# SDU-Gary/PCSS-Unet

Hardware: AMD Instinct MI355X
Metric: frames/sec 7x512x512 U-Net fwd+bwd (train step) (higher is better)
Workload: dtype f32; 1 GPU; configs[1]: batch=8/GPU 7x512x512 fp32 train step (fwd + 0.9*L1 + bwd + RCCL grad all-reduce + clip + AdamW); global_batch=8, in_ch=7, parallelism=dp1

## Files before the change

include/nsm.h:

```cpp
#ifndef NSM_H_
#define NSM_H_

#include <stddef.h>
#include <stdint.h>

#ifdef __cplusplus
extern "C" {
#endif

#define NSM_OK 0
#define NSM_E_ARG 1
#define NSM_E_HIP 2
#define NSM_E_WS 3

#define NSM_F32 0
#define NSM_BF16 1
#define NSM_F16 2

#define NSM_AMAX_WORDS 2048
#define NSM_PACK_FWD 0
#define NSM_PACK_DGRAD 1

int nsm_version(void);
int nsm_get_last_error(char* buf, size_t n);
// ... 62 lines not shown
int nsm_wino_output_bf16(const float* Mb, int B, int H, int W, int cout_p, int tile,
                         const float* bias, void* y, int ldy, float* partial, int nslot,
                         void* stream);
int nsm_wino_dual_f16(const void* dy, int lddy, int B, int H, int W, int c_p, int tile, void* V,
                      void* dM, const uint32_t* amax_dy, void* stream);
int nsm_wino_dual_bn_f16(const void* g, int ldg, const void* y, int ldy, int B, int H, int W, int c_p,
                         int tile, const float* scale, const float* shift, float slope,
                         const float* mask, const float* mean, const float* coef, void* V, void* dM,
                         const uint32_t* bound, void* stream);
int nsm_wino_gemm_f16m(const void* V, const void* U, int B, int H, int W, int cin_p, int cout_p,
                       int tile, void* M16, int* m16e, const uint32_t* amax_v, float beta_v,
                       const uint32_t* amax_u, float beta_u, void* stream);
int nsm_wino_output_bf16m(const void* M16, const int* m16e, int B, int H, int W, int cin_p,
                          int cout_p, int tile, const uint32_t* amax_v, float beta_v,
                          const uint32_t* amax_u, float beta_u, const float* bias, void* y, int ldy,
                          float* partial, int nslot, void* stream);
int nsm_wino_output_bf16m_act(const void* M16, const int* m16e, int B, int H, int W, int cin_p,
                              int cout_p, int tile, const uint32_t* amax_v, float beta_v,
                              const uint32_t* amax_u, float beta_u, const float* bias, void* y,
                              int ldy, const float* act_scale, const float* act_shift, float slope,
                              void* stream);
int nsm_wino_dout_f16(const void* dy, int lddy, int B, int H, int W, int c_p, int tile, void* dM,
                      const uint32_t* amax_dy, void* stream);
size_t nsm_wino_wgrad_f16_ws(int B, int H, int W, int cin_p, int cout_p, int tile);
int nsm_conv3x3_wgrad_wino_f16(const void* dM, const void* V, int B, int H, int W, int cin_p,
                               int cout_p, int cin, int cout, int tile, float* dw, float* ws,
                               size_t ws_floats, const uint32_t* amax_dy, const uint32_t* amax_x,
                               void* stream);
int nsm_wino_dual_input_bn_h2(const float* g, int ldg, const float* y, int ldy, int B, int H, int W,
                              int c_p, int tile, const float* scale, const float* shift,
                              float slope, const float* mask, const float* mean, const float* coef,
                              void* Vh, void* dMh, const uint32_t* bound, void* stream);
size_t nsm_wino_wgrad_h2_ws(int B, int H, int W, int cin_p, int cout_p, int tile);
int nsm_conv3x3_wgrad_wino_h2(const void* dMh, const void* Vh, int B, int H, int W, int cin_p,
                              int cout_p, int cin, int cout, int tile, float* dw, float* ws,
                              size_t ws_floats, const uint32_t* amax_dy, const uint32_t* amax_x,
                              void* stream);
int nsm_wino_gemm_h2(const void* V, const void* U, int B, int H, int W, int cin_p, int cout_p,
                     int tile, float* Mb, const uint32_t* amax_v, float beta_v,
                     const uint32_t* amax_u, float beta_u, void* stream);
int nsm_wino_gemm_h2_plan(int B, int H, int W, int cin_p, int cout_p, int tile, int* plan);
int nsm_wino_wgrad_h2_plan(int B, int H, int W, int cin_p, int cout_p, int tile, int* plan);
int nsm_conv1x1_h2_rows(int M, int N, int K, int bnbwd);
int nsm_conv1x1_h2(const void* xh, int M, int cin_p, const void* wh, const float* bias, int cout_p,
                   float* y, int ldy, float* stats, const uint32_t* amax_x,
                   const uint32_t* amax_w, void* stream);
int nsm_conv1x1_dgrad_bnbwd_h2(const void* dy2h, int M, int cop, const void* w2dh, int cip,
                               const float* y1, int ldy1, const float* scale, const float* shift,
                               const float* mean, const float* invstd, const float* mask, int HW,
                               float slope, int mode, float* partial, const float* coef,
                               float* out, int ldo, const uint32_t* amax_dy2,
                               const uint32_t* amax_w, uint32_t* amax_out, uint32_t* amax_k1dz,
                               void* stream);
size_t nsm_conv1x1_wgrad_h2_ws(int M, int cin_p, int cout_p);
int nsm_conv1x1_wgrad_h2(const void* dyh, const void* xh, int M, int cin_p, int cout_p, int cin,
                         int cout, float* dw, float* ws, size_t ws_floats, const uint32_t* amax_dy,
                         const uint32_t* amax_x, void* stream);
int nsm_conv3x3_h2_rows(int M, int N);
int nsm_conv3x3_h2(const void* xh, int B, int H, int W, int cin_p, const void* wh,
                   const float* bias, int cout_p, float* y, int ldy, float* stats,
                   const uint32_t* amax_x, const uint32_t* amax_w, void* stream);
size_t nsm_conv3x3_wgrad_h2_ws(int B, int H, int W, int cin_p, int cout_p);
int nsm_conv3x3_wgrad_h2(const void* dyh, const void* xh, int B, int H, int W, int cin_p,
                         int cout_p, int cin, int cout, float* dw, float* ws, size_t ws_floats,
                         const uint32_t* amax_dy, const uint32_t* amax_x, void* stream);
int nsm_set_f32_split(int mode);
int nsm_wino_output(const float* Mb, int B, int H, int W, int cout_p, int tile, const float* bias,
                    float* y, int ldy, void* stream);
int nsm_wino_output_stats(const float* Mb, int B, int H, int W, int cout_p, int tile,
                          const float* bias, float* y, int ldy, float* partial, int nslot,
                          void* stream);
int nsm_wino_stat_slots(int B, int H, int W, int cout_p, int tile);
int nsm_wino_stat_step(int cout_p, int tile);

size_t nsm_wino_wgrad_ws(int B, int H, int W, int cin_p, int cout_p, int tile);
int nsm_conv3x3_wgrad_wino(const float* dy, int lddy, const float* V, int B, int H, int W,
                           int cin_p, int cout_p, int cin, int cout, int tile, float* dw,
                           float* ws, size_t ws_floats, void* stream);
int nsm_wino_dual_input(const float* dy, int lddy, int B, int H, int W, int c_p, int tile,
                        float* V, float* dM, uint32_t* amax_v, uint32_t* amax_dm, void* stream);
int nsm_wino_dual_input_bn(const float* g, int ldg, const float* y, int ldy, int B, int H, int W,
                           int c_p, int tile, const float* scale, const float* shift, float slope,
                           const float* mask, const float* mean, const float* coef, float* V,
                           float* dM, uint32_t* amax_v, uint32_t* amax_dm, void* stream);
int nsm_conv3x3_wgrad_wino_dm(const float* dM, const float* V, int B, int H, int W, int cin_p,
                              int cout_p, int cin, int cout, int tile, float* dw, float* ws,
                              size_t ws_floats, const uint32_t* amax_dm, const uint32_t* amax_v,
                              void* stream);

size_t nsm_conv_wgrad_ws(int B, int H, int W, int cin_p, int cout_p, int ksize);
int nsm_conv_wgrad(const float* dy, int lddy, const float* x, int ldx, int B, int H, int W,
                   int cin_p, int cout_p, int ksize, const float* pro_scale, const float* pro_shift,
                   const float* pro_mask, float slope, float* ws, size_t ws_floats, int cin, int cout,
                   float* dw, const uint32_t* amax_dy, const uint32_t* amax_x, void* stream);

int nsm_reduce_chunks(int M, int C);
int nsm_reduce_rows(int M, int C);
int nsm_bn_stats(const void* y, int ld, int M, int C, float* partial, int nchunk, int dtype,
                 void* stream);
int nsm_bn_finalize_train(const float* partial, int nchunk, int rows_per_chunk, int M, int C,
                          int c_real,
                          const float* gamma, const float* beta, float* run_mean, float* run_var,
                          int64_t* num_batches, float momentum, float eps, int n_updates,
                          float* mean, float* invstd, float* scale, float* shift, uint32_t* bound,
                          float bound_mul, void* stream);
int nsm_bn_partials_merge(const float* partial, int nchunk, int rows_per_chunk, int M, int C,
// ... 296 lines not shown
```

pcss-unet_amd/csrc/nsm_conv_h2d.inc:

```

struct EpiStoreH {
  using P = EpiStoreP;
  template <int TM, int TN, int WM, int WN>
  static constexpr int lds_bytes() {
    constexpr int a = WM * WN * 32 * (TN * 32 + 4) * 4, b = WM * WN * TN * 32 * 4;
    return a > b ? a : b;
  }
  template <int TM, int TN, int WM, int WN>
  __device__ static void apply(const P& e, f32x16 (&acc)[TM][TN], const EpiCtx& cx, int M, int N,
                               int) {
    const int col = cx.lane & 31, h = cx.lane >> 5;
#pragma unroll
    for (int tn = 0; tn < TN; ++tn) {
      const int n = cx.nb + tn * 32 + col;
      const float bv = (e.bias && n < N) ? e.bias[n] : 0.f;
#pragma unroll
      for (int tm = 0; tm < TM; ++tm)
#pragma unroll
        for (int i = 0; i < 16; ++i) acc[tm][tn][i] += bv;
    }
    constexpr int WC = TN * 32, WCP = WC + 4, CPR = WC / 4;
    float* reg = cx.lds + (cx.wm * WN + cx.wn) * (32 * WCP);
#pragma unroll
    for (int tm = 0; tm < TM; ++tm) {
// ... 46 lines not shown
static bool h2d_nfast() { static const bool v = env_flag("NSM_H2D_NFAST", true); return v; }

template <int BM, int BN, int WM, int WN, class EP>
static int launch_h2d(const H2RowsP& ap, const H2RowsP& bp, const typename EP::P& ep, int M, int N,
                      int K, H2Scale sa, H2Scale sb, hipStream_t s) {
  constexpr int NW = WM * WN;
  const dim3 grid(ceil_div(M, BM), ceil_div(N, BN), 1);
  const long long total = (long long)grid.x * grid.y;
  const int remap = h2d_nfast() && grid.y > 1 && total % 8 == 0 ? 2 : 0;
  hipLaunchKernelGGL((gemm_h2_kernel<BM, BN, WM, WN, H2RowsDma<BM, NW>, H2RowsDma<BN, NW>, EP>), grid,
                     dim3(NW * 64), 0, s, ap, bp, ep, M, N, K, K, 1, remap, sa, sb);
  NSM_LAUNCH_CHECK("conv1x1_h2");
  return 0;
}

template <class EP>
static int gemm_h2d(int tile, const H2RowsP& ap, const H2RowsP& bp, const typename EP::P& ep, int M,
                    int N, int K, H2Scale sa, H2Scale sb, hipStream_t s) {
  switch (tile) {
    case 1:
      if constexpr (!std::is_same<EP, EpiBnBwd>::value)
        return launch_h2d<256, 256, 2, 4, EP>(ap, bp, ep, M, N, K, sa, sb, s);
      return fail(NSM_E_ARG, "conv1x1_h2: tile");
    case 2: return launch_h2d<256, 128, 4, 2, EP>(ap, bp, ep, M, N, K, sa, sb, s);
    case 3: return launch_h2d<128, 128, 2, 2, EP>(ap, bp, ep, M, N, K, sa, sb, s);
    case 4: return launch_h2d<256, 64, 4, 1, EP>(ap, bp, ep, M, N, K, sa, sb, s);
    case 5: return launch_h2d<128, 64, 2, 2, EP>(ap, bp, ep, M, N, K, sa, sb, s);
    default: return launch_h2d<128, 32, 4, 1, EP>(ap, bp, ep, M, N, K, sa, sb, s);
  }
}

static WgradPlan plan_wgrad_h2(long long px, int cin_p, int cout_p) {
  WgradPlan pl;
  pl.BM = cout_p >= 128 ? 128 : (cout_p >= 64 ? 64 : 32);
  pl.BN = cin_p >= 128 ? 128 : (cin_p >= 64 ? 64 : 32);
  const long long tiles = (long long)ceil_div(cout_p, pl.BM) * ceil_div(cin_p, pl.BN);
  static const long long target = env_int("NSM_H2D_WG_BLOCKS", 512);
  long long sp = target / tiles;
  const long long maxs = (px + 255) / 256;
  long long slab_cap = (128ll << 20) / ((long long)cout_p * cin_p);
  if (slab_cap < 1) slab_cap = 1;
  if (sp > maxs) sp = maxs;
  if (sp > slab_cap) sp = slab_cap;
  if (sp > 512) sp = 512;
  if (sp < 1) sp = 1;
  long long kc = (px + sp - 1) / sp;
  kc = (kc + 31) / 32 * 32;
  sp = (px + kc - 1) / kc;
  pl.splits = (int)sp;
  pl.kchunk = (int)kc;
  pl.ws_floats = (size_t)sp * cout_p * cin_p;
  if (sp > 16) pl.ws_floats += (size_t)((sp + 15) / 16) * cout_p * cin_p;
  return pl;
}

extern "C" int nsm_conv1x1_h2_rows(int M, int N, int K, int bnbwd) {
  return h2d_tile_bm(h2d_tile(M, N, K, bnbwd != 0));
}

extern "C" int nsm_conv1x1_h2(const void* xh, int M, int cin_p, const void* wh, const float* bias,
                              int cout_p, float* y, int ldy, float* stats, const uint32_t* amax_x,
                              const uint32_t* amax_w, void* stream) {
  NSM_CHECK_ARG(xh && wh && y && amax_x && amax_w, "conv1x1_h2: null pointer");
  NSM_CHECK_ARG(M > 0 && cin_p % 32 == 0 && cout_p % 32 == 0 && ldy >= cout_p && ldy % 4 == 0,
                "conv1x1_h2: bad shape");
  NSM_CHECK_ARG(((uintptr_t)xh % 16) == 0 && ((uintptr_t)wh % 16) == 0 && ((uintptr_t)y % 16) == 0,
                "conv1x1_h2: 16-B alignment");
  NSM_CHECK_ARG((long long)M * 2 * cin_p < (1ll << 30), "conv1x1_h2: operand too large");
  const int K = 2 * cin_p;
  H2RowsP ap{(const bf16_t*)xh, K, M, 0};
  H2RowsP bp{(const bf16_t*)wh, K, cout_p, 0};
  EpiStoreP ep{y, ldy, bias, stats, 0, nullptr, nullptr, 0.f, nullptr, 0, 1};
  return gemm_h2d<EpiStoreH>(h2d_tile(M, cout_p, K, false), ap, bp, ep, M, cout_p, K,
                             H2Scale{amax_x, 1.f}, H2Scale{amax_w, 1.f}, as_stream(stream));
}

extern "C" int nsm_conv1x1_dgrad_bnbwd_h2(const void* dy2h, int M, int cop, const void* w2dh,
                                          int cip, const float* y1, int ldy1, const float* scale,
                                          const float* shift, const float* mean,
                                          const float* invstd, const float* mask, int HW,
                                          float slope, int mode, float* partial, const float* coef,
                                          float* out, int ldo, const uint32_t* amax_dy2,
                                          const uint32_t* amax_w, uint32_t* amax_out,
                                          uint32_t* amax_k1dz, void* stream) {
  NSM_CHECK_ARG(dy2h && w2dh && y1 && scale && shift && mean && amax_dy2 && amax_w,
                "conv1x1_dgrad_bnbwd_h2: null pointer");
  NSM_CHECK_ARG(mode >= 0 && mode <= 2, "conv1x1_dgrad_bnbwd_h2: mode %d", mode);
  NSM_CHECK_ARG(mode == 2 || (partial && invstd), "conv1x1_dgrad_bnbwd_h2: modes 0/1 need partials");
  NSM_CHECK_ARG(mode == 0 || out, "conv1x1_dgrad_bnbwd_h2: modes 1/2 need an output");
  NSM_CHECK_ARG(mode != 2 || coef, "conv1x1_dgrad_bnbwd_h2: mode 2 needs coef");
  NSM_CHECK_ARG(M > 0 && HW > 0 && cop % 32 == 0 && cip % 32 == 0 && ldy1 >= cip && ldy1 % 4 == 0 &&
                    (mode == 0 || (ldo >= cip && ldo % 4 == 0)),
                "conv1x1_dgrad_bnbwd_h2: bad shape");
  NSM_CHECK_ARG(((uintptr_t)dy2h % 16) == 0 && ((uintptr_t)w2dh % 16) == 0 &&
                    ((uintptr_t)y1 % 16) == 0 && ((uintptr_t)out % 16) == 0,
                "conv1x1_dgrad_bnbwd_h2: 16-B alignment");
  NSM_CHECK_ARG((long long)M * 2 * cop < (1ll << 30), "conv1x1_dgrad_bnbwd_h2: operand too large");
  BnBwdEpiP ep{out, ldo, y1, ldy1, scale, shift, mean, invstd, coef, mask,
               make_fastdiv((uint32_t)HW), slope, partial, mode};
  if (mode == 2) ep.amax = amax_out;
  else ep.k1dz = amax_k1dz;
  const int K = 2 * cop;
  H2RowsP ap{(const bf16_t*)dy2h, K, M, 0};
  H2RowsP bp{(const bf16_t*)w2dh, K, cip, 0};
  return gemm_h2d<EpiBnBwd>(h2d_tile(M, cip, K, true), ap, bp, ep, M, cip, K, H2Scale{amax_dy2, 1.f},
                            H2Scale{amax_w, 1.f}, as_stream(stream));
}

extern "C" size_t nsm_conv1x1_wgrad_h2_ws(int M, int cin_p, int cout_p) {
  return plan_wgrad_h2(M, cin_p, cout_p).ws_floats;
}

extern "C" int nsm_conv1x1_wgrad_h2(const void* dyh, const void* xh, int M, int cin_p, int cout_p,
                                    int cin, int cout, float* dw, float* ws, size_t ws_floats,
                                    const uint32_t* amax_dy, const uint32_t* amax_x, void* stream) {
  NSM_CHECK_ARG(dyh && xh && dw && ws && amax_dy && amax_x, "conv1x1_wgrad_h2: null pointer");
  NSM_CHECK_ARG(M > 0 && cin_p % 32 == 0 && cout_p % 32 == 0 && cin <= cin_p && cout <= cout_p,
                "conv1x1_wgrad_h2: bad shape");
  NSM_CHECK_ARG(((uintptr_t)dyh % 16) == 0 && ((uintptr_t)xh % 16) == 0 && ((uintptr_t)ws % 16) == 0,
                "conv1x1_wgrad_h2: 16-B alignment");
  NSM_CHECK_ARG((long long)M * 2 * std::max(cin_p, cout_p) < (1ll << 30),
                "conv1x1_wgrad_h2: operand too large");
  const WgradPlan pl = plan_wgrad_h2(M, cin_p, cout_p);
  if (ws_floats < pl.ws_floats)
    return fail(NSM_E_WS, "conv1x1_wgrad_h2: workspace %zu < %zu floats", ws_floats, pl.ws_floats);
  hipStream_t s = as_stream(stream);
  const int rc = wino_wgrad_gemm_h2((const bf16_t*)dyh, (const bf16_t*)xh, M, cin_p, cout_p, 1,
                                    pl.BM, pl.BN, pl.kchunk, pl.splits, ws, H2Scale{amax_dy, 1.f},
                                    H2Scale{amax_x, 1.f}, s);
  if (rc) return rc;
  return wgrad_finish(ws, pl, cout_p, cin_p, cin_p, 1, cin, cout, dw, s);
}

template <int R, int NW>
struct H2ConvDma : ConvActDma<R, NW, 64> {
  static constexpr int KT = 64;
  __device__ void init(const ConvActPB& p, int m0, int kb, int ke, int wid, int lane, int) {
    ConvActDma<R, NW, 64>::init(p, m0, kb, ke, wid, lane);
  }
};
template <int R, int NW>
struct H2RowsKDma : RowsKDma<R, NW, 64> {
  static constexpr int KT = 64;
  __device__ void init(const RowsKPB& p, int n0, int kb, int ke, int wid, int lane, int) {
    RowsKDma<R, NW, 64>::init(p, n0, kb, ke, wid, lane);
  }
};
template <int R, int NW>
struct H2ShiftDma : PixRowsDma<R, NW, true, 32> {
  static constexpr int KT = 32;
  int kb0;
  __device__ void init(const PixRowsPB& p, int off, int kb, int ke, int wid, int lane, int) {
    kb0 = kb;
    PixRowsDma<R, NW, true, 32>::init(p, 2 * off, kb, ke, wid, lane);
  }
  __device__ void prep(const PixRowsPB& p, int krel) { PixRowsDma<R, NW, true, 32>::prep(p, kb0 + krel); }
};

static ConvActPB h2_conv_operand(const void* xh, int B, int H, int W, int cin_p) {
// ... 114 lines not shown
```

pcss-unet_amd/nsm_amd/_lib.py:

```python
import ctypes
import os

import torch

_HERE = os.path.dirname(os.path.abspath(__file__))
LIB_PATH = os.environ.get("NSM_LIB", os.path.join(_HERE, "libnsm.so"))

P = ctypes.c_void_p
I = ctypes.c_int
L = ctypes.c_int64
F = ctypes.c_float
Z = ctypes.c_size_t
D = ctypes.c_double
U64 = ctypes.c_uint64

_SIGS = {
    "nsm_version": (I, []),
    "nsm_get_last_error": (I, [ctypes.c_char_p, Z]),
    "nsm_pack_conv_weight": (I, [P, I, I, I, I, I, I, P, P]),
    "nsm_pad_vec": (I, [P, I, I, P, P]),
    "nsm_conv_fwd": (I, [P, I, I, I, I, I, P, P, I, I, P, I, P, P, P, F, P]),
    "nsm_conv_stat_rows": (I, [I, I, I, I]),
    "nsm_conv_fwd_stats": (I, [P, I, I, I, I, I, P, P, I, I, P, I, P, P, P, F, P, P, P, P]),
    "nsm_wino_ws": (Z, [I, I, I, I, I, I]),
    "nsm_wino_weight": (I, [P, I, I, I, I, I, I, P, P]),
    "nsm_conv3x3_wino": (I, [P, I, I, I, I, I, P, P, I, I, I, P, I, P, Z, P]),
    "nsm_wino_input": (I, [P, I, I, I, I, I, I, I, P, P]),
    "nsm_wino_gemm": (I, [P, P, I, I, I, I, I, I, P, P]),
    "nsm_wino_gemm_s": (I, [P, P, I, I, I, I, I, I, P, P, P, P]),
    "nsm_absmax": (I, [P, L, P, P]),
    "nsm_zero_u32": (I, [P, L, P]),
    "nsm_absmax_bf16": (I, [P, L, P, P]),
    "nsm_pmc_calib": (I, [I, P, P, L, P]),
    "nsm_to_h2": (I, [P, L, I, P, F, P, P]),
    "nsm_wino_gemm_h2": (I, [P, P, I, I, I, I, I, I, P, P, F, P, F, P]),
    "nsm_wino_gemm_h2_plan": (I, [I, I, I, I, I, I, P]),
    "nsm_wino_wgrad_h2_plan": (I, [I, I, I, I, I, I, P]),
    "nsm_wino_beta": (F, [I, I]),
    "nsm_wino_input_h2": (I, [P, I, I, I, I, I, I, I, I, P, P, P]),
    "nsm_wino_dual_input_h2": (I, [P, I, I, I, I, I, I, P, P, P, P]),
    "nsm_wino_dual_input_bn_h2": (I, [P, I, P, I, I, I, I, I, I, P, P, F, P, P, P, P, P, P, P]),
    "nsm_wino_input_f16": (I, [P, I, I, I, I, I, I, P, P, P]),
    "nsm_wino_input_f16_resize": (I, [P, I, I, I, I, I, I, I, I, P, P, P]),
    "nsm_wino_gemm_f16": (I, [P, P, I, I, I, I, I, I, P, P, F, P, F, P]),
    "nsm_wino_output_bf16": (I, [P, I, I, I, I, I, P, P, I, P, I, P]),
    "nsm_wino_gemm_f16m": (I, [P, P, I, I, I, I, I, I, P, P, P, F, P, F, P]),
    "nsm_wino_output_bf16m": (I, [P, P, I, I, I, I, I, I, P, F, P, F, P, P, I, P, I, P]),
    "nsm_wino_output_bf16m_act": (I, [P, P, I, I, I, I, I, I, P, F, P, F, P, P, I, P, P, F, P]),
    "nsm_wino_dout_f16": (I, [P, I, I, I, I, I, I, P, P, P]),
    "nsm_wino_dual_f16": (I, [P, I, I, I, I, I, I, P, P, P, P]),
    "nsm_wino_dual_bn_f16": (I, [P, I, P, I, I, I, I, I, I, P, P, F, P, P, P, P, P, P, P]),
    "nsm_wino_wgrad_f16_ws": (Z, [I, I, I, I, I, I]),
    "nsm_conv3x3_wgrad_wino_f16": (I, [P, P, I, I, I, I, I, I, I, I, P, P, Z, P, P, P]),
    "nsm_wino_wgrad_h2_ws": (Z, [I, I, I, I, I, I]),
    "nsm_conv3x3_wgrad_wino_h2": (I, [P, P, I, I, I, I, I, I, I, I, P, P, Z, P, P, P]),
    "nsm_set_f32_split": (I, [I]),
    "nsm_wino_output": (I, [P, I, I, I, I, I, P, P, I, P]),
    "nsm_wino_wgrad_ws": (Z, [I, I, I, I, I, I]),
    "nsm_conv3x3_wgrad_wino": (I, [P, I, P, I, I, I, I, I, I, I, I, P, P, Z, P]),
    "nsm_conv_wgrad_ws": (Z, [I, I, I, I, I, I]),
    "nsm_conv_wgrad": (I, [P, I, P, I, I, I, I, I, I, I, P, P, P, F, P, Z, I, I, P, P, P, P]),
    "nsm_reduce_chunks": (I, [I, I]),
    "nsm_reduce_rows": (I, [I, I]),
    "nsm_bn_stats": (I, [P, I, I, I, P, I, I, P]),
    "nsm_bn_finalize_train": (I, [P, I, I, I, I, I, P, P, P, P, P, F, F, I, P, P, P, P, P, F, P]),
    "nsm_bn_act_h2": (I, [P, I, I, I, P, P, F, P, I, P, P, P]),
    "nsm_conv1x1_h2_rows": (I, [I, I, I, I]),
    "nsm_conv1x1_h2": (I, [P, I, I, P, P, I, P, I, P, P, P, P]),
    "nsm_conv1x1_dgrad_bnbwd_h2": (I, [P, I, I, P, I, P, I, P, P, P, P, P, I, F, I, P, P, P, I, P,
                                       P, P, P, P]),
    "nsm_conv3x3_h2_rows": (I, [I, I]),
    "nsm_conv3x3_h2": (I, [P, I, I, I, I, P, P, I, P, I, P, P, P, P]),
    "nsm_conv3x3_wgrad_h2_ws": (Z, [I, I, I, I, I]),
    "nsm_conv3x3_wgrad_h2": (I, [P, P, I, I, I, I, I, I, I, P, P, Z, P, P, P]),
    "nsm_input_prep_h2": (I, [P, I, I, I, I, P, I, P, P]),
    "nsm_conv1x1_wgrad_h2_ws": (Z, [I, I, I]),
    "nsm_conv1x1_wgrad_h2": (I, [P, P, I, I, I, I, I, P, P, Z, P, P, P]),
    "nsm_bn_partials_merge": (I, [P, I, I, I, I, I, P, P]),
    "nsm_bn_finalize_eval": (I, [P, P, P, P, I, I, F, P, P, P, P, P]),
    "nsm_bn_act": (I, [P, I, I, I, P, P, F, P, I, P, I, P, I, I, P, P]),
    "nsm_bn_bwd_reduce": (I, [P, I, P, I, I, I, I, P, P, F, P, P, P, P, I, I, P, P]),
    "nsm_bn_bwd_finalize": (I, [P, I, I, I, I, P, P, P, P, P, P, P, P, P]),
    "nsm_bn_bwd_apply_h2": (I, [P, I, P, I, I, I, I, P, P, F, P, P, P, P, P, P]),
    "nsm_bn_bwd_apply": (I, [P, I, P, I, I, I, I, P, P, F, P, P, P, P, I, I, P, P]),
    "nsm_sum_rows": (I, [P, I, I, I, P, P]),
    "nsm_resize_fwd_act": (I, [P, I, I, I, I, P, I, I, P, P, F, P, I, P]),
    "nsm_up2_resize_fwd_act": (I, [P, I, I, I, I, P, I, I, P, P, F, P, I, P]),
    "nsm_bn_act_pool": (I, [P, I, I, I, I, P, P, F, P, P, I, P, P]),
    "nsm_wino_dual_input": (I, [P, I, I, I, I, I, I, P, P, P, P, P]),
    "nsm_wino_dual_input_bn": (I, [P, I, P, I, I, I, I, I, I, P, P, F, P, P, P, P, P, P, P, P]),
    "nsm_conv3x3_wgrad_wino_dm": (I, [P, P, I, I, I, I, I, I, I, I, P, P, Z, P, P, P]),
    "nsm_conv_fwd_act": (I, [P, I, I, I, I, I, P, P, I, I, P, I, P, P, F, P, I, I, P]),
    "nsm_wino_output_act": (I, [P, I, I, I, I, I, P, P, I, P, P, F, P, I, P]),
    "nsm_bnred_chunks": (I, [I, I, I, I, I]),
    "nsm_avgpool2_bwd_add_bnred": (I, [P, I, I, I, I, P, P, I, P, P, P, P, P, F, P, P, P]),
    "nsm_resize_bwd_bnred": (I, [P, I, I, I, I, P, I, I, I, P, P, P, P, P, F, P, P, P]),
    "nsm_up2_resize_bwd_bnred": (I, [P, I, I, I, I, P, I, I, I, P, P, P, P, P, F, P, P, P]),
    "nsm_wino_input_resize": (I, [P, I, I, I, I, I, I, I, I, I, P, P, P]),
    "nsm_wino_output_stats": (I, [P, I, I, I, I, I, P, P, I, P, I, P]),
    "nsm_wino_stat_slots": (I, [I, I, I, I, I]),
    "nsm_wino_stat_step": (I, [I, I]),
    "nsm_conv1x1_bnbwd_chunks": (I, [I, I, I, I, I, I]),
    "nsm_conv1x1_dgrad_bnbwd": (I, [P, I, I, I, I, I, P, I, P, I, P, P, P, P, P, F, I, P, P, P, I,
                                    I, P, P, P, P]),
    "nsm_avgpool2_fwd": (I, [P, I, I, I, I, P, I, P]),
    "nsm_avgpool2_bwd_add": (I, [P, I, I, I, I, P, P, I, P]),
    "nsm_resize_fwd": (I, [P, I, I, I, I, P, I, I, I, P]),
    "nsm_resize_bwd": (I, [P, I, I, I, I, P, I, I, I, P]),
    "nsm_up2_resize_fwd": (I, [P, I, I, I, I, P, I, I, I, P]),
    "nsm_up2_resize_bwd": (I, [P, I, I, I, I, P, I, I, I, P]),
    "nsm_input_prep": (I, [P, I, I, I, I, P, I, I, P, P]),
    "nsm_input_grad": (I, [P, I, I, I, I, I, P, I, P]),
    "nsm_head_fwd": (I, [P, I, I, I, I, P, P, P, I, P]),
    "nsm_head_bwd_blocks": (I, [I, I, I]),
    "nsm_head_bwd": (I, [P, P, P, I, I, I, I, P, P, P, P, P, I, P]),
    "nsm_loss_blocks": (I, [L]),
    "nsm_l1_loss_fwd": (I, [P, P, L, F, P, P, P]),
    "nsm_expdiff_mean": (I, [P, P, L, F, P, P, P]),
    "nsm_l1_loss_bwd": (I, [P, P, L, F, P, P, I, P]),
    "nsm_detail_blocks": (I, [I, I, I]),
    "nsm_detail_loss_fwd": (I, [P, P, I, I, I, F, F, F, P, P, P, P]),
    "nsm_detail_loss_bwd": (I, [P, P, I, I, I, F, F, F, P, P, P, I, P]),
    "nsm_ssim_blocks": (I, [I, I, I]),
# ... 133 lines not shown
```

pcss-unet_amd/nsm_amd/ops.py:

```python
import os

import torch

from ._lib import call, ptr, stream

F32 = torch.float32
BF16 = torch.bfloat16
F16S = torch.int16
PACK_FWD, PACK_DGRAD = 0, 1
NSM_F32, NSM_BF16, NSM_F16 = 0, 1, 2
S16 = (BF16, F16S)


def dt(t):
    if t.dtype == BF16:
        return NSM_BF16
    if t.dtype == F16S:
        return NSM_F16
    if t.dtype != F32:
        raise TypeError(f"activations must be float32, bfloat16 or f16 storage (int16), "
                        f"got {t.dtype}")
    return NSM_F32


# ... 312 lines not shown
             ptr(amax[0]), bv, ptr(amax[1]), bu, st)
    else:
        call("nsm_wino_gemm_f16", ptr(V), ptr(U), B, H, W, cin_p, cout_p, 4, ptr(Mb), ptr(amax[0]),
             bv, ptr(amax[1]), bu, st)
    if evg is not None:
        evg.record()
    if not keep_v:
        V = None
    y = torch.empty(B * H * W, cout_p, dtype=BF16, device=x.device)
    if act is not None:
        assert not stats
        call("nsm_wino_output_bf16m_act", ptr(Mb), ptr(m16e), B, H, W, cin_p, cout_p, 4,
             ptr(amax[0]), bv, ptr(amax[1]), bu, ptr(bias), ptr(y), y.stride(0), ptr(act.scale),
             ptr(act.shift), 0.2, st)
        if ev is not None:
            ev.record()
        return (y, None, V) if keep_v else (y, None)
    nslot = int(lib.nsm_wino_stat_slots(B, H, W, cout_p, 4)) if stats else 0
    part = None
    if nslot > 0:
        part = Partials(empty(nslot * 3 * cout_p, device=x.device), nslot, 0)
    pb = ptr(part.buf) if part is not None else None
    if m16:
        call("nsm_wino_output_bf16m", ptr(Mb), ptr(m16e), B, H, W, cin_p, cout_p, 4, ptr(amax[0]),
             bv, ptr(amax[1]), bu, ptr(bias), ptr(y), y.stride(0), pb, nslot, st)
    else:
        call("nsm_wino_output_bf16", ptr(Mb), B, H, W, cout_p, 4, ptr(bias), ptr(y), y.stride(0),
             pb, nslot, st)
    if ev is not None:
        ev.record()
    return (y, part, V) if keep_v else (y, part)


H2 = torch.float16
_BETA = {}


def wino_beta(tile, which):
    key = (tile, which)
    if key not in _BETA:
        from ._lib import lib
        _BETA[key] = float(lib.nsm_wino_beta(tile, which))
    return _BETA[key]


H2_GEMM_FORMS = ("gemm_h2", "gemm_h2q", "gemm_h2p")


def wino_gemm_h2_plan(B, H, W, cin_p, cout_p, tile):
    import ctypes
    plan = (ctypes.c_int * 2)()
    call("nsm_wino_gemm_h2_plan", B, H, W, cin_p, cout_p, tile, plan)
    return plan[0], H2_GEMM_FORMS[plan[1]]


def wino_wgrad_h2_plan(B, H, W, cin_p, cout_p, tile):
    import ctypes
    plan = (ctypes.c_int * 4)()
    call("nsm_wino_wgrad_h2_plan", B, H, W, cin_p, cout_p, tile, plan)
    return tuple(plan)


def wino_dual_input_h2(dy, B, H, W, tile, amax_dy):
    c_p = dy.shape[1]
    n = (tile + 2) ** 2 * wino_tiles(B, H, W, tile) * 2 * c_p
    Vd = torch.empty(n, dtype=H2, device=dy.device)
    dM = torch.empty(n, dtype=H2, device=dy.device)
    call("nsm_wino_dual_input_h2", ptr(dy), dy.stride(0), B, H, W, c_p, tile, ptr(Vd), ptr(dM),
         ptr(amax_dy), stream())
    return Vd, dM


def wino_dual_input(dy, B, H, W, tile=4, amax=(None, None)):
    c_p = dy.shape[1]
    n = (tile + 2) ** 2 * wino_tiles(B, H, W, tile) * c_p
    Vd = empty(n, device=dy.device)
    dM = empty(n, device=dy.device)
    call("nsm_wino_dual_input", ptr(dy), dy.stride(0), B, H, W, c_p, tile, ptr(Vd), ptr(dM),
         ptr(amax[0]), ptr(amax[1]), stream())
    return Vd, dM


class DeferredBnBwd:
    __slots__ = ("g", "coef", "shape", "device", "dtype")

    def __init__(self, g, coef):
        self.g, self.coef = g, coef
        self.shape, self.device, self.dtype = g.shape, g.device, g.dtype


def wino_dual_input_bn(d, y, st, mask, B, H, W, tile=4, slope=0.2, amax=(None, None)):
    c_p = y.shape[1]
    n = (tile + 2) ** 2 * wino_tiles(B, H, W, tile) * c_p
    Vd = empty(n, device=y.device)
    dM = empty(n, device=y.device)
    call("nsm_wino_dual_input_bn", ptr(d.g), d.g.stride(0), ptr(y), y.stride(0), B, H, W, c_p,
         tile, ptr(st.scale), ptr(st.shift), slope, ptr(mask), ptr(st.mean), ptr(d.coef),
         ptr(Vd), ptr(dM), ptr(amax[0]), ptr(amax[1]), stream())
    return Vd, dM


def wino_dual_input_bn_h2(d, y, st, mask, B, H, W, tile, bound, slope=0.2):
    c_p = y.shape[1]
    n = (tile + 2) ** 2 * wino_tiles(B, H, W, tile) * 2 * c_p
    Vd = torch.empty(n, dtype=H2, device=y.device)
    dM = torch.empty(n, dtype=H2, device=y.device)
# ... 599 lines not shown
```

Measured before the change: 770.8 frames/s.

## Add persistent double-buffered kernel for 1x1 dgrad with fused BN-backward epilogue

Adds a persistent GEMM kernel for the 1x1 conv dgrad that has the BN-backward epilogue fused in. Each block walks several output tiles in a swizzled order and prefetches the next tile's A/B operands and Y activations while the current tile's MFMAs and epilogue are still running. The goal is to hide per-tile prologue and epilogue latency and cut launch and tail imbalance on large grids. A policy picks it when the tile count exceeds the CU count, and env and API knobs can override that; the cost is more complexity and a fixed occupancy of 2 waves per EU.

```diff
diff --git a/include/nsm.h b/include/nsm.h
--- a/include/nsm.h
+++ b/include/nsm.h
@@ -138,6 +138,9 @@
                                float* out, int ldo, const uint32_t* amax_dy2,
                                const uint32_t* amax_w, uint32_t* amax_out, uint32_t* amax_k1dz,
                                void* stream);
+int nsm_set_h2d_bnb_persist(int form, int grid, int* prev);
+int nsm_conv1x1_dgrad_bnbwd_h2_plan(int M, int cip, int cop, int* plan);
+int nsm_h2d_tile_walk(int gx, int gy, int grid, int block, int* out, int cap, int* count);
 size_t nsm_conv1x1_wgrad_h2_ws(int M, int cin_p, int cout_p);
 int nsm_conv1x1_wgrad_h2(const void* dyh, const void* xh, int M, int cin_p, int cout_p, int cin,
                          int cout, float* dw, float* ws, size_t ws_floats, const uint32_t* amax_dy,
diff --git a/pcss-unet_amd/csrc/nsm_conv_h2d.inc b/pcss-unet_amd/csrc/nsm_conv_h2d.inc
--- a/pcss-unet_amd/csrc/nsm_conv_h2d.inc
+++ b/pcss-unet_amd/csrc/nsm_conv_h2d.inc
@@ -122,6 +122,318 @@
   pl.ws_floats = (size_t)sp * cout_p * cin_p;
   if (sp > 16) pl.ws_floats += (size_t)((sp + 15) / 16) * cout_p * cin_p;
   return pl;
+}
+
+__host__ __device__ inline int h2d_tile_decode(int L, int gx, int gy, int& m, int& n) {
+  const int total = gx * gy;
+  const int lg = (gy > 1 && (total & 7) == 0) ? (L & 7) * (total >> 3) + (L >> 3) : L;
+  m = lg / gy;
+  n = lg - m * gy;
+  return lg;
+}
+
+template <int BM, int BN, int WM, int WN>
+__global__ void __launch_bounds__(WM * WN * 64) __attribute__((amdgpu_waves_per_eu(2, 2)))
+    gemm_h2bp_kernel(H2RowsP ap, H2RowsP bp, BnBwdEpiP ep, int M, int N, int K, int gx, int gy,
+                     H2Scale sca, H2Scale scb) {
+  constexpr int NW = WM * WN, TM = BM / (WM * 32), TN = BN / (WN * 32);
+  static_assert(TM == 2 && TN == 2, "64 x 64 wave tiles");
+  using AL = H2RowsDma<BM, NW>;
+  using BL = H2RowsDma<BN, NW>;
+  constexpr int KT = 64;
+  constexpr int A_EL = BM * KT, STAGE = (BM + BN) * KT;
+  constexpr int LPT = AL::NI + BL::NI;
+  constexpr int CPR = 16, NIT = 16;
+  constexpr int SLAB = 16 * 64;
+  static_assert(LPT <= 63 && 2 * NIT <= 63, "vmcnt range");
+  __shared__ __attribute__((aligned(1024))) bf16_t lds[2 * STAGE + 2 * NW * SLAB];
+
+  const int total = gx * gy;
+  int L = blockIdx.x;
+  if (L >= total) return;
+  const int tid = threadIdx.x, lane = tid & 63;
+  const int wid = __builtin_amdgcn_readfirstlane(tid >> 6);
+  const int wm = wid / WN, wn = wid % WN;
+  const int nk = K / KT;
+  const float ia = exp2i(-h2_exp(sca)), ib = exp2i(-h2_exp(scb));
+  int bm, bn;
+  h2d_tile_decode(L, gx, gy, bm, bn);
+
+  const int arb = wm * TM * 32, brb = wn * TN * 32;
+  const int cc = lane % CPR, rq = lane / CPR;
+  const float* __restrict__ Y = (const float*)ep.y;
+  f32x4 yv[NIT];
+#pragma unroll
+  for (int it = 0; it < NIT; ++it) {
+    const int m = min(bm * BM + arb + it * 4 + rq, M - 1);
+    yv[it] = *(const f32x4*)(Y + (size_t)m * ep.ldy + bn * BN + brb + cc * 4);
+  }
+
+  AL a;
+  BL b;
+  a.rows(ap, wid, lane);
+  b.rows(bp, wid, lane);
+  a.aim(ap, bm * BM, 0);
+  b.aim(bp, bn * BN, 0);
+  a.prep(ap, 0);
+  b.prep(bp, 0);
+#pragma unroll
+  for (int j = 0; j < LPT; ++j) dma_one(a, b, ap, bp, lds, A_EL, wid, j);
+  a.prep(ap, KT);
+  b.prep(bp, KT);
+#pragma unroll
+  for (int j = 0; j < LPT; ++j) dma_one(a, b, ap, bp, lds + STAGE, A_EL, wid, j);
+  vm_wait<0>();
+  dma_barrier();
+
+  using FR = FragH2<false, KT>;
+  FR fa[2][2][TM];
+  FR fb[2][2][TN];
+#pragma unroll
+  for (int p = 0; p < 2; ++p) {
+#pragma unroll
+    for (int tm = 0; tm < TM; ++tm) fa[0][p][tm].issue(lds, arb + tm * 32, lane, 0, p);
+#pragma unroll
+    for (int tn = 0; tn < TN; ++tn) fb[0][p][tn].issue(lds + A_EL, brb + tn * 32, lane, 0, p);
+  }
+  const __amdgpu_buffer_rsrc_t orsrc =
+      __builtin_amdgcn_make_buffer_rsrc(ep.out, (short)0, ep.out ? M * ep.ldo * 4 : 0, 0x00020000);
+  float* const stg = (float*)(lds + 2 * STAGE) + wid * SLAB;
+  const float* const stg0 = (const float*)(lds + 2 * STAGE);
+  const bool red = ep.mode != 2;
+  int st = 0;
+  for (; L < total; L += (int)gridDim.x) {
+    const bool has_next = L + (int)gridDim.x < total;
+    int bmn = 0, bnn = 0;
+    if (has_next) h2d_tile_decode(L + (int)gridDim.x, gx, gy, bmn, bnn);
+    f32x16 acc[TM][TN];
+#pragma unroll
+    for (int i = 0; i < TM; ++i)
+#pragma unroll
+      for (int j = 0; j < TN; ++j)
+#pragma unroll
+        for (int e = 0; e < 16; ++e) acc[i][j][e] = 0.f;
+    for (int t = 0; t < nk; ++t) {
+      const bf16_t* As = lds + st * STAGE;
+      const bf16_t* Bs = As + A_EL;
+#pragma unroll
+      for (int p = 0; p < 2; ++p) {
+#pragma unroll
+        for (int tm = 0; tm < TM; ++tm) fa[1][p][tm].issue(As, arb + tm * 32, lane, 1, p);
+#pragma unroll
+        for (int tn = 0; tn < TN; ++tn) fb[1][p][tn].issue(Bs, brb + tn * 32, lane, 1, p);
+      }
+      __builtin_amdgcn_s_setprio(1);
+#pragma unroll
+      for (int tm = 0; tm < TM; ++tm)
+#pragma unroll
+        for (int tn = 0; tn < TN; ++tn) mfma_h2<TM, TN>(acc, fa[0], fb[0], tm, tn);
+      __builtin_amdgcn_s_setprio(0);
+      const int tgt = t + 2;
+      const bool more = t + 1 < nk || has_next, refill = tgt < nk || has_next;
+      if (refill) {
+        if (tgt < nk) {
+          a.prep(ap, tgt * KT);
+          b.prep(bp, tgt * KT);
+        } else {
+          if (tgt == nk) {
+            a.aim(ap, bmn * BM, 0);
+            b.aim(bp, bnn * BN, 0);
+          }
+          a.prep(ap, (tgt - nk) * KT);
+          b.prep(bp, (tgt - nk) * KT);
+        }
+      }
+      __builtin_amdgcn_s_waitcnt(0xC07F);
+      if (more) {
+        int tq = t;
+        asm volatile("" : "+s"(tq));
+        if (tq == 0) {
+          if (ep.mode == 0) vm_wait<NIT>();
+          else vm_wait<2 * NIT>();
+        } else {
+          vm_wait<0>();
+        }
+        __builtin_amdgcn_s_barrier();
+        const bf16_t* Ns = lds + (st ^ 1) * STAGE;
+#pragma unroll
+        for (int p = 0; p < 2; ++p) {
+#pragma unroll
+          for (int tm = 0; tm < TM; ++tm) fa[0][p][tm].issue(Ns, arb + tm * 32, lane, 0, p);
+#pragma unroll
+          for (int tn = 0; tn < TN; ++tn) fb[0][p][tn].issue(Ns + A_EL, brb + tn * 32, lane, 0, p);
+        }
+      }
+      __builtin_amdgcn_s_setprio(1);
+#pragma unroll
+      for (int tm = 0; tm < TM; ++tm)
+#pragma unroll
+        for (int tn = 0; tn < TN; ++tn) {
+          mfma_h2<TM, TN>(acc, fa[1], fb[1], tm, tn);
+          if (refill) {
+            const int q = tm * TN + tn;
+#pragma unroll
+            for (int i = 0; i < LPT; ++i)
+              if (i * (TM * TN) / LPT == q) dma_one(a, b, ap, bp, As, A_EL, wid, i);
+          }
+        }
+      __builtin_amdgcn_s_setprio(0);
+      st ^= 1;
+    }
+
+    int el = lane;
+    asm volatile("" : "+v"(el));
+    const int col = el & 31, h = el >> 5;
+    const int ec = el % CPR, er = el / CPR;
+    const int mb = bm * BM + arb, n = bn * BN + brb + ec * 4;
+    const int mbn = bmn * BM + arb, nn = bnn * BN + brb + ec * 4;
+    const float* __restrict__ mk = ep.mask;
+    const f32x4 sc = *(const f32x4*)(ep.scale + n), sh = *(const f32x4*)(ep.shift + n),
+                mu = *(const f32x4*)(ep.mean + n);
+    const f32x4 zero = {0.f, 0.f, 0.f, 0.f};
+    const f32x4 is = red ? *(const f32x4*)(ep.invstd + n) : zero;
+    const f32x4 k1 = red ? zero : *(const f32x4*)(ep.coef + n),
+                k2 = red ? zero : *(const f32x4*)(ep.coef + N + n),
+                k3 = red ? zero : *(const f32x4*)(ep.coef + 2 * N + n);
+    const bool mrow = mk && ep.fdHW.d < 64u;
+    f32x4 mk0 = zero, mk1 = zero;
+    int mth = 0;
+    if (mk && !mrow) {
+      const uint32_t b0 = fdiv((uint32_t)min(mb, M - 1), ep.fdHW),
+                     b1 = fdiv((uint32_t)min(mb + 63, M - 1), ep.fdHW);
+      mk0 = *(const f32x4*)(mk + (size_t)b0 * N + n);
+      mk1 = *(const f32x4*)(mk + (size_t)b1 * N + n);
+      mth = (int)((b0 + 1u) * ep.fdHW.d);
+    }
+    asm volatile("" ::"v"(sc), "v"(sh), "v"(mu), "v"(is), "v"(k1), "v"(k2), "v"(k3), "v"(mk0), "v"(mk1));
+    f32x4 s1 = zero, s2 = zero;
+    uint32_t am = 0;
+#pragma unroll
+    for (int sl = 0; sl < 4; ++sl) {
+      const int tm = sl >> 1, hf = sl & 1;
+#pragma unroll
+      for (int tn = 0; tn < TN; ++tn)
+#pragma unroll
+        for (int j = 0; j < 8; ++j)
+          stg[((j & 3) + 8 * (j >> 2) + 4 * h) * 64 + tn * 32 + col] = (acc[tm][tn][8 * hf + j] * ia) * ib;
+      __builtin_amdgcn_fence(__ATOMIC_RELEASE, "wavefront");
+      __builtin_amdgcn_wave_barrier();
+      __builtin_amdgcn_fence(__ATOMIC_ACQUIRE, "wavefront");
+#pragma unroll
+      for (int q = 0; q < 4; ++q) {
+        const int it = sl * 4 + q;
+        const int m = mb + it * 4 + er;
+        const bool ok = m < M;
+        const uint32_t ooff = ok ? (uint32_t)(m * ep.ldo + n) * 4u : OOB;
+        const f32x4 g = *(const f32x4*)&stg[(q * 4 + er) * 64 + ec * 4], v = yv[it];
+        f32x4 dz = g * lrelu_grad_v4(v * sc + sh, ep.slope);
+        if (mrow) dz = dz * *(const f32x4*)(mk + (size_t)fdiv((uint32_t)min(m, M - 1), ep.fdHW) * N + n);
+        else if (mk) dz = dz * (m < mth ? mk0 : mk1);
+        if (!red) {
+          const f32x4 d = k1 * dz + k2 * (v - mu) + k3;
+          uint32_t a2 = am;
+          amax_fold(a2, d);
+          am = ok ? a2 : am;
+          __builtin_amdgcn_raw_buffer_store_b128(__builtin_bit_cast(u32x4, d), orsrc, ooff, 0, 0);
+        } else {
+          const f32x4 t1 = s1 + dz, t2 = s2 + dz * ((v - mu) * is);
+          s1 = ok ? t1 : s1;
+          s2 = ok ? t2 : s2;
+          if (ep.k1dz) {
+            uint32_t a2 = am;
+            amax_fold(a2, sc * dz);
+            am = ok ? a2 : am;
+          }
+          if (ep.mode == 1)
+            __builtin_amdgcn_raw_buffer_store_b128(__builtin_bit_cast(u32x4, g), orsrc, ooff, 0, 0);
+        }
+      }
+      if (has_next) {
+#pragma unroll
+        for (int q = 0; q < 4; ++q) {
+          const int it = sl * 4 + q;
+          const int m = min(mbn + it * 4 + er, M - 1);
+          yv[it] = *(const f32x4*)(Y + (size_t)m * ep.ldy + nn);
+        }
+      }
+      __builtin_amdgcn_fence(__ATOMIC_RELEASE, "wavefront");
+      __builtin_amdgcn_wave_barrier();
+      __builtin_amdgcn_fence(__ATOMIC_ACQUIRE, "wavefront");
+    }
+    uint32_t* const aslot = red ? ep.k1dz : ep.amax;
+    if (aslot) {
+#pragma unroll
+      for (int o = 32; o > 0; o >>= 1) am = max(am, (uint32_t)__shfl_xor((int)am, o));
+      const uint32_t line = ((uint32_t)bm + 7u * (uint32_t)bn) & (AMAX_LINES - 1);
+      if (el == 0 && am) atomicMax(aslot + line * AMAX_STRIDE, am);
+    }
+    if (red) {
+#pragma unroll
+      for (int o = CPR; o < 64; o <<= 1) {
+        s1 += shfl_xor_v4(s1, o);
+        s2 += shfl_xor_v4(s2, o);
+      }
+      if (el < CPR) {
+        *(f32x4*)(stg + ec * 4) = s1;
+        *(f32x4*)(stg + 64 + ec * 4) = s2;
+      }
+      dma_barrier();
+      if (wm == 0) {
+        float* pr = ep.partial + (size_t)bm * 2 * N;
+        for (int j = el; j < 2 * 64; j += 64) {
+          const int k = j / 64, c = j - k * 64;
+          float t = 0.f;
+#pragma unroll
+          for (int w = 0; w < WM; ++w) t += stg0[(w * WN + wn) * SLAB + k * 64 + c];
+          pr[k * N + bn * BN + brb + c] = t;
+        }
+      }
+    }
+    bm = bmn;
+    bn = bnn;
+  }
+}
+
+static int g_h2d_bnb_form = [] {
+  const long long v = env_int("NSM_H2D_BNB_PERSIST", 1);
+  return v == 0 ? 1 : v == 2 ? 2 : 0;
+}();
+static int g_h2d_bnb_grid = 0;
+
+static bool h2d_bnb_covered(int tile, long long M, int N, int K, int ldo) {
+  return (tile == 2 || tile == 3) && N % 128 == 0 && K % 64 == 0 && K >= 128 &&
+         M * (long long)std::max(ldo, N) * 4 < (1ll << 31) &&
+         ceil_div(M, h2d_tile_bm(tile)) * (N / 128) < (1ll << 30);
+}
+static bool h2d_bnb_persistent(int tile, long long M, int N, int K, int ldo) {
+  if (g_h2d_bnb_form == 1 || !h2d_bnb_covered(tile, M, N, K, ldo)) return false;
+  if (g_h2d_bnb_form == 2) return true;
+  const long long tiles = ceil_div(M, h2d_tile_bm(tile)) * (N / 128);
+  return tiles > (long long)cu_count() * (tile == 3 ? 2 : 1);
+}
+
+template <int BM, int BN, int WM, int WN>
+static int h2bp_grid(long long total) {
+  static const int resident = [] {
+    int occ = 0;
+    if (hipOccupancyMaxActiveBlocksPerMultiprocessor(&occ, gemm_h2bp_kernel<BM, BN, WM, WN>,
+                                                     WM * WN * 64, 0) != hipSuccess || occ < 1)
+      occ = 1;
+    return std::min(occ, 2) * cu_count();
+  }();
+  const long long g = g_h2d_bnb_grid > 0 ? g_h2d_bnb_grid : resident;
+  return (int)std::min<long long>(g, total);
+}
+
+template <int BM, int BN, int WM, int WN>
+static int launch_h2bp(const H2RowsP& ap, const H2RowsP& bp, const BnBwdEpiP& ep, int M, int N, int K,
+                       H2Scale sa, H2Scale sb, hipStream_t s) {
+  const int gx = ceil_div(M, BM), gy = N / BN;
+  const int grid = h2bp_grid<BM, BN, WM, WN>((long long)gx * gy);
+  hipLaunchKernelGGL((gemm_h2bp_kernel<BM, BN, WM, WN>), dim3(grid), dim3(WM * WN * 64), 0, s, ap, bp,
+                     ep, M, N, K, gx, gy, sa, sb);
+  NSM_LAUNCH_CHECK("conv1x1_h2 (persistent)");
+  return 0;
 }
 
 extern "C" int nsm_conv1x1_h2_rows(int M, int N, int K, int bnbwd) {
@@ -173,8 +485,57 @@
   const int K = 2 * cop;
   H2RowsP ap{(const bf16_t*)dy2h, K, M, 0};
   H2RowsP bp{(const bf16_t*)w2dh, K, cip, 0};
-  return gemm_h2d<EpiBnBwd>(h2d_tile(M, cip, K, true), ap, bp, ep, M, cip, K, H2Scale{amax_dy2, 1.f},
+  const int tile = h2d_tile(M, cip, K, true);
+  if (h2d_bnb_persistent(tile, M, cip, K, mode == 0 ? cip : ldo)) {
+    if (tile == 2)
+      return launch_h2bp<256, 128, 4, 2>(ap, bp, ep, M, cip, K, H2Scale{amax_dy2, 1.f},
+                                         H2Scale{amax_w, 1.f}, as_stream(stream));
+    return launch_h2bp<128, 128, 2, 2>(ap, bp, ep, M, cip, K, H2Scale{amax_dy2, 1.f},
+                                       H2Scale{amax_w, 1.f}, as_stream(stream));
+  }
+  return gemm_h2d<EpiBnBwd>(tile, ap, bp, ep, M, cip, K, H2Scale{amax_dy2, 1.f},
                             H2Scale{amax_w, 1.f}, as_stream(stream));
+}
+
+extern "C" int nsm_set_h2d_bnb_persist(int form, int grid, int* prev) {
+  NSM_CHECK_ARG(form <= 2, "set_h2d_bnb_persist: form %d", form);
+  if (prev) {
+    prev[0] = g_h2d_bnb_form;
+    prev[1] = g_h2d_bnb_grid;
+  }
+  if (form >= 0) g_h2d_bnb_form = form;
+  if (grid >= 0) g_h2d_bnb_grid = grid;
+  return 0;
+}
+
+extern "C" int nsm_conv1x1_dgrad_bnbwd_h2_plan(int M, int cip, int cop, int* plan) {
+  NSM_CHECK_ARG(plan && M > 0 && cip > 0 && cop > 0 && cip % 32 == 0 && cop % 32 == 0,
+                "conv1x1_dgrad_bnbwd_h2_plan: bad args");
+  const int K = 2 * cop, tile = h2d_tile(M, cip, K, true), bm = h2d_tile_bm(tile);
+  const bool p = h2d_bnb_persistent(tile, M, cip, K, cip);
+  const long long total = (long long)ceil_div(M, bm) * ceil_div(cip, 128);
+  plan[0] = tile;
+  plan[1] = p ? 1 : 0;
+  plan[2] = !p ? 0 : tile == 2 ? h2bp_grid<256, 128, 4, 2>(total) : h2bp_grid<128, 128, 2, 2>(total);
+  plan[3] = bm;
+  return 0;
+}
+
+extern "C" int nsm_h2d_tile_walk(int gx, int gy, int grid, int block, int* out, int cap,
+                                 int* count) {
+  NSM_CHECK_ARG(out && count && gx > 0 && gy > 0 && grid > 0 && block >= 0 && block < grid &&
+                    cap >= 0 && (long long)gx * gy < (1ll << 30),
+                "h2d_tile_walk: bad args");
+  int cnt = 0;
+  for (int L = block; L < gx * gy; L += grid, ++cnt) {
+    if (cnt >= cap) continue;
+    int m, n;
+    out[3 * cnt + 2] = h2d_tile_decode(L, gx, gy, m, n);
+    out[3 * cnt] = m;
+    out[3 * cnt + 1] = n;
+  }
+  *count = cnt;
+  return 0;
 }
 
 extern "C" size_t nsm_conv1x1_wgrad_h2_ws(int M, int cin_p, int cout_p) {
diff --git a/pcss-unet_amd/nsm_amd/_lib.py b/pcss-unet_amd/nsm_amd/_lib.py
--- a/pcss-unet_amd/nsm_amd/_lib.py
+++ b/pcss-unet_amd/nsm_amd/_lib.py
@@ -69,6 +69,9 @@
     "nsm_conv1x1_h2": (I, [P, I, I, P, P, I, P, I, P, P, P, P]),
     "nsm_conv1x1_dgrad_bnbwd_h2": (I, [P, I, I, P, I, P, I, P, P, P, P, P, I, F, I, P, P, P, I, P,
                                        P, P, P, P]),
+    "nsm_set_h2d_bnb_persist": (I, [I, I, P]),
+    "nsm_conv1x1_dgrad_bnbwd_h2_plan": (I, [I, I, I, P]),
+    "nsm_h2d_tile_walk": (I, [I, I, I, I, P, I, P]),
     "nsm_conv3x3_h2_rows": (I, [I, I]),
     "nsm_conv3x3_h2": (I, [P, I, I, I, I, P, P, I, P, I, P, P, P, P]),
     "nsm_conv3x3_wgrad_h2_ws": (Z, [I, I, I, I, I]),
diff --git a/pcss-unet_amd/nsm_amd/ops.py b/pcss-unet_amd/nsm_amd/ops.py
--- a/pcss-unet_amd/nsm_amd/ops.py
+++ b/pcss-unet_amd/nsm_amd/ops.py
@@ -388,6 +388,35 @@
     plan = (ctypes.c_int * 2)()
     call("nsm_wino_gemm_h2_plan", B, H, W, cin_p, cout_p, tile, plan)
     return plan[0], H2_GEMM_FORMS[plan[1]]
+
+
+H2D_BNB_FORMS = ("policy", "old", "persistent")
+
+
+def set_h2d_bnb_persist(form=-1, grid=-1):
+    import ctypes
+    if isinstance(form, str):
+        form = H2D_BNB_FORMS.index(form)
+    prev = (ctypes.c_int * 2)()
+    call("nsm_set_h2d_bnb_persist", int(form), int(grid), prev)
+    return prev[0], prev[1]
+
+
+def conv1x1_dgrad_bnbwd_h2_plan(M, cip, cop):
+    import ctypes
+    plan = (ctypes.c_int * 4)()
+    call("nsm_conv1x1_dgrad_bnbwd_h2_plan", M, cip, cop, plan)
+    return plan[0], ("old", "persistent")[plan[1]], plan[2], plan[3]
+
+
+def h2d_tile_walk(gx, gy, grid, block):
+    import ctypes
+    cap = -(-gx * gy // grid)
+    out = (ctypes.c_int * (3 * max(cap, 1)))()
+    cnt = ctypes.c_int(0)
+    call("nsm_h2d_tile_walk", gx, gy, grid, block, out, cap, ctypes.byref(cnt))
+    assert cnt.value <= cap
+    return [(out[3 * i], out[3 * i + 1], out[3 * i + 2]) for i in range(cnt.value)]
 
 
 def wino_wgrad_h2_plan(B, H, W, cin_p, cout_p, tile):
```

After: 780.8 frames/s, median of 6. 1.01x the previous value.
